# ysbbin/Robust-Object-Detection

Measured on NVIDIA B200. Metric: corrupted images/sec (1360x765 RGB), motion blur k=9, higher is better.
Workload: dtype u8

## Files before the change

robust-object-detection_b200/csrc/api.cu:

```cuda
#include <algorithm>
#include <vector>

#include "rod_internal.h"
#include "rod_tables.h"

using namespace rod;

namespace {

constexpr float kPhiloxMaxSigma = 2048.0f;

bool blur_supported(int k, double angle) { return angle == 0.0 && k >= 1 && k <= 31 && (k & 1) == 1; }

int run_op(rod_plan* plan, int op, const uint8_t* src, uint8_t* dst, const float* noise, float sigma, int k,
           double factor, uint64_t seed, uint64_t first_image, uint32_t offset, const uint8_t* opcodes,
           cudaStream_t stream, int img_lo, int img_hi) {
    switch (op) {
        case ROD_OP_NONE:
            return launch_noise(plan, NOISE_COPY, src, dst, nullptr, nullptr, 0.f, 0, 0, 0, opcodes, ROD_OP_NONE,
                                stream, img_lo, img_hi);
        case ROD_OP_NOISE:
            if (noise == nullptr && sigma > kPhiloxMaxSigma) return ROD_ERR_UNSUPPORTED;
            return launch_noise(plan, noise ? NOISE_COMPAT : NOISE_PHILOX, src, dst, noise, nullptr, sigma, seed,
                                first_image, offset, opcodes, ROD_OP_NOISE, stream, img_lo, img_hi);
        case ROD_OP_BLUR:
            if (plan->f2d_ntaps > 0) return launch_filter2d(plan, src, dst, opcodes, stream, img_lo, img_hi);
            if (!blur_supported(k, 0.0)) return ROD_ERR_UNSUPPORTED;
            if (k == 1)
                return launch_noise(plan, NOISE_COPY, src, dst, nullptr, nullptr, 0.f, 0, 0, 0, opcodes, ROD_OP_BLUR,
                                    stream, img_lo, img_hi);
            return launch_blur(plan, src, dst, k, opcodes, stream, img_lo, img_hi);
        case ROD_OP_LOWRES: {
            int rc = ensure_lowres_tables(plan, factor);
            if (rc != ROD_OK) return rc;
            if (plan->lowres_all_identity)
                return launch_noise(plan, NOISE_COPY, src, dst, nullptr, nullptr, 0.f, 0, 0, 0, opcodes,
                                    ROD_OP_LOWRES, stream, img_lo, img_hi);
            return launch_lowres(plan, src, dst, opcodes, stream, img_lo, img_hi);
        }
        default:
            return ROD_ERR_INVALID_ARG;
    }
}

int run_mixed_ops(rod_plan* plan, int op_lo, const uint8_t* src, uint8_t* dst, const uint8_t* opcodes, const float* noise,
                  float sigma, int k, double factor, uint64_t seed, uint64_t first_image, uint32_t offset,
                  cudaStream_t stream) {
    if (noise == nullptr && sigma > kPhiloxMaxSigma) return ROD_ERR_UNSUPPORTED;
    if (plan->f2d_ntaps == 0 && !blur_supported(k, 0.0)) return ROD_ERR_UNSUPPORTED;
    {
        const int rc = ensure_lowres_tables(plan, factor);
        if (rc != ROD_OK) return rc;
    }
    const bool fork = plan->n_images <= 128;
    if (fork && plan->ev_fork == nullptr) {
        cudaStream_t s2[2] = {nullptr, nullptr};
        cudaEvent_t ef = nullptr, ej[2] = {nullptr, nullptr};
        cudaError_t e = cudaSuccess;
        for (auto& s : s2)
            if (e == cudaSuccess) e = cudaStreamCreateWithFlags(&s, cudaStreamNonBlocking);
        if (e == cudaSuccess) e = cudaEventCreateWithFlags(&ef, cudaEventDisableTiming);
        for (auto& ev : ej)
            if (e == cudaSuccess) e = cudaEventCreateWithFlags(&ev, cudaEventDisableTiming);
        if (e != cudaSuccess) {
            for (auto& s : s2) if (s) cudaStreamDestroy(s);
            if (ef) cudaEventDestroy(ef);
            for (auto& ev : ej) if (ev) cudaEventDestroy(ev);
            return cuda_fail(e);
        }
        plan->aux_streams[0] = s2[0]; plan->aux_streams[1] = s2[1];
        plan->ev_join[0] = ej[0]; plan->ev_join[1] = ej[1];
        plan->ev_fork = ef;
    }
    if (fork) {
        ROD_CUDA(cudaEventRecord(plan->ev_fork, stream));
        for (auto& s : plan->aux_streams) ROD_CUDA(cudaStreamWaitEvent(s, plan->ev_fork, 0));
    }
    int first_rc = ROD_OK;
    for (int op = op_lo; op <= ROD_OP_LOWRES && first_rc == ROD_OK; ++op) {
        cudaStream_t st = stream;
        if (fork && op == ROD_OP_BLUR) st = plan->aux_streams[0];
        if (fork && op == ROD_OP_NOISE) st = plan->aux_streams[1];
        first_rc = run_op(plan, op, src, dst, noise, sigma, k, factor, seed, first_image, offset, opcodes, st, 0, plan->n_images);
    }
    if (fork) {
        for (int i = 0; i < 2; ++i) {
            cudaError_t e = cudaEventRecord(plan->ev_join[i], plan->aux_streams[i]);
            if (e == cudaSuccess) e = cudaStreamWaitEvent(stream, plan->ev_join[i], 0);
            if (e != cudaSuccess && first_rc == ROD_OK) first_rc = cuda_fail(e);
        }
    }
    return first_rc;
}

}

extern "C" const char* rod_version(void) { return "rod_b200 0.1.0 (sm_100a)"; }

extern "C" int rod_device_count(void) {
    int n = 0;
    if (cudaGetDeviceCount(&n) != cudaSuccess) {
        cudaGetLastError();
        return 0;
    }
    return n;
}

extern "C" int rod_last_cuda_error(void) { return g_last_cuda_error; }

extern "C" const char* rod_status_string(int status) {
    switch (status) {
        case ROD_OK: return "ok";
        case ROD_ERR_INVALID_ARG: return "invalid argument";
        case ROD_ERR_UNSUPPORTED: return "parameter outside the exact-parity domain (no approximation, no CPU fallback)";
        case ROD_ERR_CUDA: return "CUDA error";
        case ROD_ERR_NO_DEVICE: return "no CUDA device (there is no CPU fallback)";
        case ROD_ERR_OOM: return "out of memory";
        default: return "unknown status";
    }
}

extern "C" int rod_plan_launches(const rod_plan* plan, int op) {
    if (plan == nullptr) return 0;
    switch (op) {
        case ROD_OP_NONE: case ROD_OP_NOISE: case ROD_OP_BLUR: return 1;
        case ROD_OP_LOWRES: {
            if (plan->d_shapes == nullptr) return 1;
            int n = 0;
            for (int l = 0; l < LR_NUM_LISTS; ++l) n += l != LR_X2_STRIP && plan->lowres[l].n > 0;
            return n > 0 ? n : 1;
        }
        case 100: return 4;
        case 101: return 4;
        default: return 0;
    }
}

extern "C" int rod_noise_u8(const rod_plan* plan, const uint8_t* src, uint8_t* dst, const float* noise, float sigma,
                            uint64_t seed, uint64_t first_image_index, uint32_t offset, const uint8_t* opcodes,
                            void* stream) {
    if (plan == nullptr || src == nullptr || dst == nullptr) return ROD_ERR_INVALID_ARG;
    if (!(sigma >= 0.0f)) return ROD_ERR_INVALID_ARG;
    if (noise == nullptr && sigma > kPhiloxMaxSigma) return ROD_ERR_UNSUPPORTED;
    return launch_noise(plan, noise ? NOISE_COMPAT : NOISE_PHILOX, src, dst, noise, nullptr, sigma, seed,
                        first_image_index, offset, opcodes, ROD_OP_NOISE, (cudaStream_t)stream, 0, plan->n_images);
}

extern "C" int rod_noise_prewarm(int device, float sigma) {
    if (!(sigma >= ROD_GAUSS_TABLE_MIN_SIGMA && sigma <= ROD_GAUSS_TABLE_MAX_SIGMA)) return ROD_OK;
    int prev = 0;
    ROD_CUDA(cudaGetDevice(&prev));
    ROD_CUDA(cudaSetDevice(device));
    const int32_t* t = nullptr;
    const int rc = rod::gauss_table_for(device, sigma, &t);
    cudaSetDevice(prev);
    return rc;
}

extern "C" int rod_gauss_table_i32(float sigma, int32_t* out256) {
    if (out256 == nullptr || !(sigma >= ROD_GAUSS_TABLE_MIN_SIGMA && sigma <= ROD_GAUSS_TABLE_MAX_SIGMA)) return ROD_ERR_INVALID_ARG;
    rod::build_gauss_table(sigma, out256);
    return ROD_OK;
}

extern "C" int rod_plan_set_gaussian_generator(rod_plan* plan, int generator) {
    if (plan == nullptr || (generator != ROD_GAUSS_AUTO && generator != ROD_GAUSS_BOXMULLER && generator != ROD_GAUSS_TABLE_PHILOX7)) return ROD_ERR_INVALID_ARG;
    plan->gauss_generator = generator;
    if (plan->inner != nullptr) plan->inner->gauss_generator = generator;
    return ROD_OK;
}

extern "C" int rod_noise_field_f32(const rod_plan* plan, float* out_field, float sigma, uint64_t seed,
                                   uint64_t first_image_index, uint32_t offset, void* stream) {
    if (plan == nullptr || out_field == nullptr) return ROD_ERR_INVALID_ARG;
    if (!(sigma >= 0.0f) || sigma > kPhiloxMaxSigma) return ROD_ERR_UNSUPPORTED;
    return launch_noise(plan, NOISE_FIELD, nullptr, nullptr, nullptr, out_field, sigma, seed, first_image_index,
                        offset, nullptr, ROD_OP_NOISE, (cudaStream_t)stream, 0, plan->n_images);
}

extern "C" int rod_blur_h_u8(const rod_plan* plan, const uint8_t* src, uint8_t* dst, int k, double angle_deg,
                             const uint8_t* opcodes, void* stream) {
    if (plan == nullptr || src == nullptr || dst == nullptr) return ROD_ERR_INVALID_ARG;
    if (plan->f2d_ntaps > 0 ? (k != plan->f2d_k) : !blur_supported(k, angle_deg)) return ROD_ERR_UNSUPPORTED;
    return run_op(const_cast<rod_plan*>(plan), ROD_OP_BLUR, src, dst, nullptr, 0.f, k, 0.0, 0, 0, 0, opcodes,
                  (cudaStream_t)stream, 0, plan->n_images);
}

extern "C" int rod_lowres_u8(rod_plan* plan, const uint8_t* src, uint8_t* dst, double factor, const uint8_t* opcodes,
                             void* stream) {
    if (plan == nullptr || src == nullptr || dst == nullptr) return ROD_ERR_INVALID_ARG;
    return run_op(plan, ROD_OP_LOWRES, src, dst, nullptr, 0.f, 0, factor, 0, 0, 0, opcodes, (cudaStream_t)stream, 0,
                  plan->n_images);
}

extern "C" int rod_corrupt_batch_u8(rod_plan* plan, const uint8_t* src, uint8_t* dst, const uint8_t* opcodes,
                                    const float* noise, float sigma, int k, double factor, uint64_t seed,
                                    uint64_t first_image_index, uint32_t offset, void* stream) {
    if (plan == nullptr || src == nullptr || dst == nullptr || opcodes == nullptr) return ROD_ERR_INVALID_ARG;
    if (noise == nullptr && sigma > kPhiloxMaxSigma) return ROD_ERR_UNSUPPORTED;
    if (plan->f2d_ntaps == 0 && !blur_supported(k, 0.0)) return ROD_ERR_UNSUPPORTED;
    int rc = ensure_lowres_tables(plan, factor);
    if (rc != ROD_OK) return rc;
    rc = run_op(plan, ROD_OP_NONE, src, dst, noise, sigma, k, factor, seed, first_image_index, offset, opcodes,
                (cudaStream_t)stream, 0, plan->n_images);
    if (rc != ROD_OK) return rc;
    return run_mixed_ops(plan, ROD_OP_NOISE, src, dst, opcodes, noise, sigma, k, factor, seed, first_image_index, offset,
                         (cudaStream_t)stream);
}

extern "C" int rod_corrupt_letterbox_f16(rod_plan* plan, const uint8_t* src, const uint8_t* opcodes, void* out_f16,
                                         int out_h, int out_w, int pad_value, const float* noise, float sigma, int k,
                                         double factor, uint64_t seed, uint64_t first_image_index, uint32_t offset,
                                         void* stream) {
    if (plan == nullptr || src == nullptr || out_f16 == nullptr || opcodes == nullptr) return ROD_ERR_INVALID_ARG;
    if (pad_value < 0 || pad_value > 255) return ROD_ERR_INVALID_ARG;
    struct GeneratorScope {
        rod_plan* p; int saved;
        explicit GeneratorScope(rod_plan* pl) : p(pl), saved(pl->gauss_generator) { p->gauss_generator = ROD_GAUSS_BOXMULLER; }
        ~GeneratorScope() { p->gauss_generator = saved; }
    } generator_scope(plan);
    int rc = ensure_letterbox_tables(plan, out_h, out_w);
    if (rc != ROD_OK) return rc;
    if (plan->d_scratch == nullptr || plan->scratch_bytes < plan->dst_extent) {
        if (plan->d_scratch) cudaFree(plan->d_scratch);
        plan->d_scratch = nullptr;
        ROD_CUDA(cudaMalloc((void**)&plan->d_scratch, plan->dst_extent + 64));
        plan->scratch_bytes = plan->dst_extent;
    }
    const bool fused = plan->lb_all_linear && plan->f2d_ntaps == 0 && blur_supported(k, 0.0) && k >= 3 &&
                       (noise != nullptr || sigma <= kPhiloxMaxSigma);
    if (fused) {
        rc = ensure_lowres_tables(plan, factor);
        if (rc != ROD_OK) return rc;
        const bool in_kernel = plan->lowres_all_x2w && (((uintptr_t)src) & 3) == 0;
        if (!in_kernel) {
            rc = run_op(plan, ROD_OP_LOWRES, src, plan->d_scratch, noise, sigma, k, factor, seed, first_image_index, offset,
                        opcodes, (cudaStream_t)stream, 0, plan->n_images);
            if (rc != ROD_OK) return rc;
        }
        rc = launch_fused_letterbox(plan, src, plan->d_scratch, opcodes, noise, out_f16, pad_value, sigma, k, seed,
                                    first_image_index, offset, in_kernel, (cudaStream_t)stream);
        if (rc != ROD_ERR_UNSUPPORTED) return rc;
    }
    rc = run_mixed_ops(plan, ROD_OP_NOISE, src, plan->d_scratch, opcodes, noise, sigma, k, factor, seed, first_image_index,
                       offset, (cudaStream_t)stream);
    if (rc != ROD_OK) return rc;
    return launch_letterbox(plan, plan->d_scratch, src, opcodes, out_f16, pad_value, (cudaStream_t)stream);
}

extern "C" int rod_resize_linear_u8(const uint8_t* src, int h, int w, int64_t src_pitch, uint8_t* dst, int nh, int nw,
                                    int64_t dst_pitch, void* stream) {
    if (src == nullptr || dst == nullptr || h < 1 || w < 1 || nh < 1 || nw < 1 || src_pitch < 3LL * w || dst_pitch < 3LL * nw ||
        h > 65535 || w > 65535 || nh > 65535 || nw > 65535)
        return ROD_ERR_INVALID_ARG;
    if (nh < h || nw < w) return ROD_ERR_UNSUPPORTED;
    return launch_resize_linear(src, h, w, src_pitch, dst, nh, nw, dst_pitch, (cudaStream_t)stream);
}

extern "C" int rod_restoration_pairs_f32(rod_plan* plan, const uint8_t* src, const uint8_t* flips, const uint8_t* opcodes,
                                         float* corrupted_out, float* clean_out, const float* noise, float sigma, int k,
                                         double factor, uint64_t seed, uint64_t first_image_index, uint32_t offset,
                                         void* stream) {
    if (plan == nullptr || src == nullptr || opcodes == nullptr || corrupted_out == nullptr || clean_out == nullptr)
        return ROD_ERR_INVALID_ARG;
    const int n = plan->n_images;
    for (int i = 1; i < n; ++i)
        if (plan->descs[i].height != plan->descs[0].height || plan->descs[i].width != plan->descs[0].width)
            return ROD_ERR_INVALID_ARG;
    if (plan->inner == nullptr) {
        std::vector<rod_image_desc> d(n);
        const uint64_t bytes = 3ull * plan->descs[0].height * plan->descs[0].width;
        const uint64_t stride = (bytes + 255) / 256 * 256;
        for (int i = 0; i < n; ++i) {
            d[i].src_offset = d[i].dst_offset = i * stride;
            d[i].height = plan->descs[0].height;
            d[i].width = plan->descs[0].width;
            d[i].src_pitch = d[i].dst_pitch = 3ll * d[i].width;
        }
// ... 114 lines not shown
```

robust-object-detection_b200/csrc/blur.cu:

```cuda

#include "rod_internal.h"

namespace rod {

struct BlurParams {
    const DevImage* images;
    const Tile* tiles;
    int n_tiles;
    const uint8_t* src;
    uint8_t* dst;
    const uint8_t* opcodes;
    int k;
    int row_buf_bytes;
    unsigned int* counter;
};

constexpr int kBlurLeft = 64;

__device__ __forceinline__ void cp_async16(uint32_t smem_addr, const void* gptr) {
    asm volatile("cp.async.cg.shared.global [%0], [%1], 16;" ::"r"(smem_addr), "l"(gptr) : "memory");
}
__device__ __forceinline__ void cp_async_wait_all() {
    asm volatile("cp.async.commit_group;\ncp.async.wait_group 0;" ::: "memory");
}
__device__ __forceinline__ void stg16_blur(void* p, uint4 v) {
    asm volatile("st.global.L1::no_allocate.v4.u32 [%0], {%1,%2,%3,%4};" ::"l"(p), "r"(v.x), "r"(v.y), "r"(v.z),
                 "r"(v.w)
                 : "memory");
}

template <int K>
__global__ void __launch_bounds__(256, 4) blur_rows_kernel(BlurParams p) {
    extern __shared__ __align__(16) uint8_t smem[];
    const int warp = threadIdx.x >> 5, lane = threadIdx.x & 31;
    uint8_t* buf = smem + (size_t)warp * p.row_buf_bytes;
    const uint32_t buf_s = (uint32_t)__cvta_generic_to_shared(buf);
    const int k = (K == 0) ? p.k : K;
    const int halo = 3 * (k >> 1);

    for (int sub = 8, ti = 0;;) {
        if (sub >= 8) {
            if (lane == 0) ti = (int)atomicAdd(p.counter, 1u);
            ti = __shfl_sync(0xFFFFFFFFu, ti, 0);
            sub = 0;
        }
        if (ti >= p.n_tiles) break;
        const Tile t = p.tiles[ti];
        const int wr = sub++;
        if (p.opcodes != nullptr && p.opcodes[t.img] != ROD_OP_BLUR) { sub = 8; continue; }
        if (wr >= t.b) { sub = 8; continue; }
        const DevImage im = p.images[t.img];
        const int y = t.a + wr;
        const int n = 3 * im.w;
        const uint8_t* srow = p.src + im.src_off + (int64_t)y * im.src_pitch;
        uint8_t* drow = p.dst + im.dst_off + (int64_t)y * im.dst_pitch;
        const int shift = (int)((uintptr_t)drow & 15);
        uint8_t* row = buf + kBlurLeft + shift;
        const int jf0 = (shift != 0) ? 1 : 0;
        const int jf1 = (n + shift) >> 4;
        const bool right_edge = ((n + shift) & 15) != 0;

        if ((((uintptr_t)srow ^ (uintptr_t)drow) & 15) == 0) {
            const uint8_t* sal = srow - shift;
            for (int j = jf0 + lane; j < jf1; j += 32) cp_async16(buf_s + kBlurLeft + 16 * j, sal + 16 * j);
            const int i = (lane < 16) ? (lane - shift) : (16 * jf1 - shift + lane - 16);
            if (((lane < 16) ? (shift != 0) : right_edge) && i >= 0 && i < n) row[i] = srow[i];
            cp_async_wait_all();
        } else {
            for (int i = lane; i < n; i += 32) row[i] = srow[i];
        }
        __syncwarp();
        if (lane < 2 * halo || K == 0) {
            for (int q = lane; q < 2 * halo; q += 32) {
                const int i = (q < halo) ? (q - halo) : (n + q - halo);
                const int px = (i >= 0) ? i / 3 : -((-i + 2) / 3);
                const int c = i - 3 * px;
                int rp;
                if (im.w > (k >> 1)) rp = (px < 0) ? -px : 2 * (im.w - 1) - px;
                else rp = reflect101(px, im.w);
                row[i] = row[3 * rp + c];
            }
        }
        __syncwarp();
        uint8_t* dal = drow - shift;
        if (K == 9) {
            for (int j = jf0 + lane; j < jf1; j += 32) {
                const uint4* wp = reinterpret_cast<const uint4*>(buf + kBlurLeft + 16 * j - 16);
                const uint4 a = wp[0], b = wp[1], c = wp[2];
                const uint32_t w[12] = {a.x, a.y, a.z, a.w, b.x, b.y, b.z, b.w, c.x, c.y, c.z, c.w};
                uint32_t out[4];
                blur9_chunk16(w, out);
                stg16_blur(dal + 16 * j, make_uint4(out[0], out[1], out[2], out[3]));
            }
            if (lane < 2 && ((lane == 0) ? (shift != 0) : right_edge)) {
                const int j = (lane == 0) ? 0 : jf1;
                const uint4* wp = reinterpret_cast<const uint4*>(buf + kBlurLeft + 16 * j - 16);
                const uint4 a = wp[0], b = wp[1], c = wp[2];
                const uint32_t w[12] = {a.x, a.y, a.z, a.w, b.x, b.y, b.z, b.w, c.x, c.y, c.z, c.w};
                uint32_t out[4];
                blur9_chunk16(w, out);
                const int lo = 16 * j - shift;
                for (int bb = 0; bb < 16; ++bb) {
                    const int i = lo + bb;
                    if (i >= 0 && i < n) drow[i] = (uint8_t)(out[bb >> 2] >> (8 * (bb & 3)));
                }
            }
        } else {
            const int nchunks = (shift + n + 15) >> 4;
            for (int j = lane; j < nchunks; j += 32) {
                const int lo = 16 * j - shift;
                uint32_t out[4];
#pragma unroll
                for (int g = 0; g < 4; ++g) {
                    uint32_t o = 0;
#pragma unroll
                    for (int b = 0; b < 4; ++b) {
                        const int i = lo + 4 * g + b;
                        const uint32_t v = (i >= 0 && i < n) ? blur_byte_generic(row, i, k) : 0u;
                        o |= v << (8 * b);
                    }
                    out[g] = o;
                }
                if (lo >= 0 && lo + 16 <= n) {
                    stg16_blur(dal + 16 * j, make_uint4(out[0], out[1], out[2], out[3]));
                } else {
                    for (int b = 0; b < 16; ++b) {
                        const int i = lo + b;
                        if (i >= 0 && i < n) drow[i] = (uint8_t)(out[b >> 2] >> (8 * (b & 3)));
                    }
                }
            }
        }
        __syncwarp();
    }
}

int launch_blur(const rod_plan* plan, const uint8_t* src, uint8_t* dst, int k, const uint8_t* opcodes,
                cudaStream_t stream, int img_lo, int img_hi) {
    const auto [tiles, n_tiles] = plan->blur_tiles.range(img_lo, img_hi);
    if (n_tiles == 0) return ROD_OK;
    BlurParams p;
    p.images = plan->d_images;
    p.tiles = tiles;
    p.n_tiles = n_tiles;
    p.src = src; p.dst = dst; p.opcodes = opcodes; p.k = k;
    const int row_bytes = 3 * plan->max_w;
    p.row_buf_bytes = kBlurLeft + ((15 + row_bytes + 15) & ~15) + 64;
    int warps = kBlurRowsPerTile;
    while (warps > 1 && (size_t)p.row_buf_bytes * warps > 227 * 1024) --warps;
    const size_t smem = (size_t)p.row_buf_bytes * warps;
    if (smem > 227 * 1024) return ROD_ERR_UNSUPPORTED;
    int ctas_per_sm = (int)((227 * 1024) / (smem + 1024));
    if (ctas_per_sm < 1) ctas_per_sm = 1;
    if (ctas_per_sm > 4) ctas_per_sm = 4;
    p.counter = plan->d_counters + (plan->launch_seq.fetch_add(1u) & (kCounterRing - 1u));
    ROD_CUDA(cudaMemsetAsync(p.counter, 0, sizeof(unsigned int), stream));
    const int grid = grid_for(plan, (p.n_tiles + warps - 1) / warps, ctas_per_sm);
    if (k == 9) {
        ROD_CUDA(cudaFuncSetAttribute(blur_rows_kernel<9>, cudaFuncAttributeMaxDynamicSharedMemorySize, (int)smem));
        blur_rows_kernel<9><<<grid, 32 * warps, smem, stream>>>(p);
    } else {
        ROD_CUDA(cudaFuncSetAttribute(blur_rows_kernel<0>, cudaFuncAttributeMaxDynamicSharedMemorySize, (int)smem));
        blur_rows_kernel<0><<<grid, 32 * warps, smem, stream>>>(p);
    }
    ROD_CUDA(cudaGetLastError());
    return ROD_OK;
}

}
```

robust-object-detection_b200/csrc/plan.cu:

```cuda
#include <map>
#include <new>

#include "rod_internal.h"
#include "rod_tables.h"

namespace rod {

thread_local int g_last_cuda_error = 0;

int grid_for(const rod_plan* plan, int n_tiles, int ctas_per_sm) {
    long long cap = (long long)plan->sm_count * ctas_per_sm;
    return (int)(n_tiles < cap ? n_tiles : cap);
}

static cudaError_t plan_alloc(const rod_plan* plan, void** p, size_t n) {
    const cudaError_t e = block_cache_alloc(plan->device, p, n);
    if (e == cudaSuccess) {
        std::lock_guard<std::mutex> lock(plan->cached_mutex);
        plan->cached_blocks.push_back({*p, n});
    }
    return e;
}
static void plan_free(const rod_plan* plan, void* p) {
    if (p == nullptr) return;
// ... 108 lines not shown
        const DevShape& sh = shapes[plan->h_images[i].shape_id];
        if (odd_image(i)) {
            std::vector<Tile>& list = lists[sh.x2i != 0 ? LR_X2I_CARRY + sh.x2i - 1 : LR_X2G];
            for (int y = 0; y < plan->h_images[i].h; y += band_rows_odd)
                for (int st = 0; st < n_strips(plan->h_images[i].w); ++st)
                    list.push_back(Tile{i, y, std::min(plan->h_images[i].h, y + band_rows_odd), st});
            continue;
        }
        if (sh.strip_rows <= 0) continue;
        if (march_image(i)) {
            const int l = packed_image(i) ? LR_X2P16 + packed_class(i) : regular_image(i) ? LR_X2H16 + packed_class(i)
                          : float_image(i) ? LR_X2F16 + packed_class(i) : al8_image(i) ? LR_X2W8 : LR_X2W4;
            for (int y = 0; y < plan->h_images[i].h; y += band_rows)
                for (int st = 0; st < n_strips(plan->h_images[i].w); ++st)
                    lists[l].push_back(Tile{i, y, std::min(plan->h_images[i].h, y + band_rows), st});
        } else {
            for (int y = 0; y < plan->h_images[i].h; y += sh.strip_rows) lists[LR_X2_REST].push_back(Tile{i, y, 0, 0});
        }
    }
    plan->lowres_factor = -1.0;
    plan_free(plan, plan->d_shapes);
    plan_free(plan, plan->d_tab);
    plan->d_shapes = nullptr;
    plan->d_tab = nullptr;
    int rc = upload(plan, shapes, &plan->d_shapes);
    if (rc == ROD_OK) rc = upload(plan, blob, &plan->d_tab);
    for (int l = 0; l < LR_NUM_LISTS && rc == ROD_OK; ++l) rc = upload_tiles(plan, lists[l], &plan->lowres[l]);
    if (rc != ROD_OK) return rc;
    plan->lowres_x2_smem = x2_smem;
    plan->lowres_factor = factor;
    plan->lowres_all_identity = all_identity;
    plan->lowres_all_x2w = true;
    for (const DevShape& sh : shapes)
        if (!sh.lin_identity && !sh.x2w) plan->lowres_all_x2w = false;
    for (int i = 0; i < plan->n_images; ++i)
        if ((plan->h_images[i].src_pitch & 3) != 0 || (plan->h_images[i].src_off & 3) != 0) plan->lowres_all_x2w = false;
    plan->lowres_half_rows = max_rows;
    plan->lowres_half_cols = max_cols;
    plan->lowres_src_rows = max_src_rows;
    return ROD_OK;
}

int ensure_letterbox_tables(rod_plan* plan, int out_h, int out_w) {
    if (plan->d_lb != nullptr && plan->lb_out_h == out_h && plan->lb_out_w == out_w) return ROD_OK;
    if (out_h < 1 || out_w < 1) return ROD_ERR_INVALID_ARG;
    std::vector<uint32_t> blob;
    std::vector<DevLetterbox> lbs(plan->shapes.size());
    for (size_t s = 0; s < plan->shapes.size(); ++s) {
        DevLetterbox g;
        memset(&g, 0, sizeof(g));
        g.h = plan->shapes[s].h; g.w = plan->shapes[s].w;
        letterbox_geometry(g.h, g.w, out_h, out_w, &g.new_h, &g.new_w, &g.top, &g.left);
        if (g.new_h < 1 || g.new_w < 1 || g.h > 65535 || g.w > 65535) return ROD_ERR_UNSUPPORTED;
        g.identity = (g.new_h == g.h && g.new_w == g.w);
        g.area2 = (!g.identity && g.h == 2 * g.new_h && g.w == 2 * g.new_w);
        if (!g.identity && !g.area2) {
            LinearAxis lx = build_linear_axis(g.w, g.new_w, true);
            LinearAxis ly = build_linear_axis(g.h, g.new_h, false);
            std::vector<uint32_t> ys(g.new_h);
            for (int y = 0; y < g.new_h; ++y) ys[y] = (uint32_t)ly.s0[y] | ((uint32_t)ly.s1[y] << 16);
            g.lx_s0 = blob_push(blob, lx.s0);
            g.lx_a = blob_push(blob, lx.coef);
            g.ly_s = blob_push(blob, ys);
            g.ly_b = blob_push(blob, ly.coef);
            std::vector<uint32_t> pack((size_t)2 * out_w);
            for (int X = 0; X < out_w; ++X) {
                const int cx = X - g.left;
                const bool in = cx >= 0 && cx < g.new_w;
                pack[2 * X] = in ? (uint32_t)(3 * lx.s0[cx]) : 0xFFFFFFFFu;
                pack[2 * X + 1] = in ? lx.coef[cx] : 0u;
            }
            g.lx_pack = blob_push(blob, pack);
            const double stride_words = 2.0 * 3.0 * ((double)g.w / (double)g.new_w) / 4.0;
            g.lane_group = 0;
            for (int pp = 2; pp <= 16; ++pp) {
                const double x = pp * stride_words / 32.0;
                if (fabs(x - nearbyint(x)) * 32.0 < 1.0) { g.lane_group = pp; break; }
            }
        }
        lbs[s] = g;
    }
    if (blob.empty()) blob.push_back(0);
    std::vector<Tile> tiles;
    for (int i = 0; i < plan->n_images; ++i)
        for (int y = 0; y < out_h; y += kLbTH)
            for (int x = 0; x < out_w; x += kLbTW) tiles.push_back(Tile{i, y, x, 0});
    if (plan->d_lb) { plan_free(plan, plan->d_lb); plan->d_lb = nullptr; }
    if (plan->d_lb_tab) { plan_free(plan, plan->d_lb_tab); plan->d_lb_tab = nullptr; }
    int rc = upload(plan, lbs, &plan->d_lb);
    if (rc != ROD_OK) return rc;
    rc = upload(plan, blob, &plan->d_lb_tab);
    if (rc != ROD_OK) return rc;
    rc = upload_tiles(plan, tiles, &plan->lb_tiles);
    if (rc != ROD_OK) return rc;
    plan->lb_all_linear = true;
    for (const DevLetterbox& g : lbs)
        if (g.identity || g.area2) plan->lb_all_linear = false;
    plan->lb_out_h = out_h;
    plan->lb_out_w = out_w;
    return ROD_OK;
}

}

using namespace rod;

extern "C" int rod_plan_create(const rod_image_desc* images, int n_images, rod_plan** out_plan) {
    if (out_plan == nullptr) return ROD_ERR_INVALID_ARG;
    *out_plan = nullptr;
    if (images == nullptr || n_images < 1) return ROD_ERR_INVALID_ARG;
    int ndev = 0;
    if (cudaGetDeviceCount(&ndev) != cudaSuccess || ndev == 0) {
        cudaGetLastError();
        return ROD_ERR_NO_DEVICE;
    }
    rod_plan* plan = new (std::nothrow) rod_plan();
    if (plan == nullptr) return ROD_ERR_OOM;
    cudaError_t e = cudaGetDevice(&plan->device);
    if (e == cudaSuccess) e = cudaDeviceGetAttribute(&plan->sm_count, cudaDevAttrMultiProcessorCount, plan->device);
    if (e != cudaSuccess) { delete plan; return cuda_fail(e); }
    plan->n_images = n_images;
    plan->descs.assign(images, images + n_images);
    plan->h_images.resize(n_images);
    std::map<std::pair<int, int>, int> shape_ids;
    uint64_t elem = 0;
    for (int i = 0; i < n_images; ++i) {
        const rod_image_desc& d = images[i];
        if (d.height < 1 || d.width < 1 || d.width > 65535 || d.height > 65535 || d.src_pitch < 3LL * d.width ||
            d.dst_pitch < 3LL * d.width || (uint64_t)d.height * d.width * 3 > 0x7FFFFFFFull) {
            delete plan;
            return ROD_ERR_INVALID_ARG;
        }
        DevImage& im = plan->h_images[i];
        im.src_off = d.src_offset; im.dst_off = d.dst_offset;
        im.src_pitch = d.src_pitch; im.dst_pitch = d.dst_pitch;
        im.h = d.height; im.w = d.width;
        im.elem_base = elem;
        im.contiguous = (d.src_pitch == 3LL * d.width && d.dst_pitch == 3LL * d.width) ? 1 : 0;
        elem += (uint64_t)d.height * d.width * 3;
        auto key = std::make_pair(d.height, d.width);
        auto it = shape_ids.find(key);
        if (it == shape_ids.end()) {
            it = shape_ids.emplace(key, (int)plan->shapes.size()).first;
            plan->shapes.push_back(HostShape{d.height, d.width});
        }
        im.shape_id = it->second;
        plan->max_w = std::max(plan->max_w, d.width);
        plan->all_contiguous = plan->all_contiguous && im.contiguous;
        plan->src_min_offset = (i == 0) ? d.src_offset : std::min<uint64_t>(plan->src_min_offset, d.src_offset);
        plan->src_extent = std::max<uint64_t>(plan->src_extent, d.src_offset + (uint64_t)(d.height - 1) * d.src_pitch + 3ull * d.width);
        plan->dst_extent = std::max<uint64_t>(plan->dst_extent, d.dst_offset + (uint64_t)(d.height - 1) * d.dst_pitch + 3ull * d.width);
    }
    plan->payload_bytes = elem;
    std::vector<Tile> nt, bt;
    build_noise_tiles(plan->h_images, kNoiseSpan, nt);
    build_blur_tiles(plan->h_images, kBlurRowsPerTile, bt);
    for (int i = 1; i < n_images; ++i) {
        const rod_image_desc& a = images[i - 1];
        const rod_image_desc& b = images[i];
        if (b.src_offset < a.src_offset + (uint64_t)a.height * a.src_pitch - (a.src_pitch - 3ull * a.width) ||
            b.dst_offset < a.dst_offset + (uint64_t)a.height * a.dst_pitch - (a.dst_pitch - 3ull * a.width))
            plan->monotonic = false;
    }
    if (plan_alloc(plan, (void**)&plan->d_counters, kCounterRing * sizeof(unsigned int)) != cudaSuccess) { rod_plan_destroy(plan); return ROD_ERR_OOM; }
    int rc = upload(plan, plan->h_images, &plan->d_images);
    if (rc == ROD_OK) rc = upload_tiles(plan, nt, &plan->noise_tiles);
    if (rc == ROD_OK) rc = upload_tiles(plan, bt, &plan->blur_tiles);
    if (rc != ROD_OK) { rod_plan_destroy(plan); return rc; }
    *out_plan = plan;
    return ROD_OK;
}

extern "C" int rod_set_blur_kernel(rod_plan* plan, const float* kernel, int k) {
    if (plan == nullptr) return ROD_ERR_INVALID_ARG;
    if (kernel == nullptr) {
        plan->f2d_ntaps = 0;
        plan->f2d_k = 0;
        return ROD_OK;
    }
    if (k < 1 || (k & 1) == 0) return ROD_ERR_INVALID_ARG;
    if (k * k >= kF2dMaxElems) return ROD_ERR_UNSUPPORTED;
    std::vector<float4> taps;
    for (int dy = 0; dy < k; ++dy)
        for (int dx = 0; dx < k; ++dx) {
            const float w = kernel[dy * k + dx];
            if (w == 0.0f) continue;
            float4 t;
            const int dxb = 3 * dx;
            memcpy(&t.x, &dy, 4);
            memcpy(&t.y, &dxb, 4);
            t.z = w;
            t.w = 0.f;
            taps.push_back(t);
        }
    if (taps.empty()) return ROD_ERR_INVALID_ARG;
    if (plan->d_f2d_taps) { plan_free(plan, plan->d_f2d_taps); plan->d_f2d_taps = nullptr; }
    int rc = upload(plan, taps, &plan->d_f2d_taps);
    if (rc != ROD_OK) return rc;
    if (plan->f2d_tiles.d == nullptr) {
        std::vector<Tile> tiles;
        build_grid_tiles(plan->h_images, kF2dTH, kF2dTWB, tiles);
        rc = upload_tiles(plan, tiles, &plan->f2d_tiles);
        if (rc != ROD_OK) return rc;
    }
    plan->f2d_ntaps = (int)taps.size();
    plan->f2d_k = k;
    return ROD_OK;
}

extern "C" void rod_plan_destroy(rod_plan* plan) {
    if (plan == nullptr) return;
    if (plan->inner) rod_plan_destroy(plan->inner);
    cudaDeviceSynchronize();
    if (plan->d_patch_clean) cudaFree(plan->d_patch_clean);
    if (plan->d_patch_corrupted) cudaFree(plan->d_patch_corrupted);
    void* ptrs[] = {plan->d_images, plan->noise_tiles.d, plan->blur_tiles.d, plan->d_shapes, plan->d_tab, plan->d_lb,
                    plan->d_lb_tab, plan->lb_tiles.d, plan->d_scratch, plan->d_stage_src, plan->d_f2d_taps,
                    plan->f2d_tiles.d, plan->d_counters, plan->d_stage_dst, plan->d_stage_noise, plan->d_stage_ops};
    for (void* p : ptrs) plan_free(plan, p);
    for (const TileList& l : plan->lowres) plan_free(plan, l.d);
    for (cudaStream_t s : plan->streams)
        if (s) cudaStreamDestroy(s);
    for (cudaStream_t s : plan->aux_streams)
        if (s) cudaStreamDestroy(s);
    for (cudaStream_t s : plan->lr_streams)
        if (s) cudaStreamDestroy(s);
    if (plan->lr_ev_fork) cudaEventDestroy(plan->lr_ev_fork);
    for (cudaEvent_t e : plan->lr_ev_join)
        if (e) cudaEventDestroy(e);
    if (plan->ev_fork) cudaEventDestroy(plan->ev_fork);
    for (cudaEvent_t e : plan->ev_join)
        if (e) cudaEventDestroy(e);
    delete plan;
}

extern "C" int rod_plan_num_images(const rod_plan* plan) { return plan ? plan->n_images : 0; }
extern "C" uint64_t rod_plan_payload_bytes(const rod_plan* plan) { return plan ? plan->payload_bytes : 0; }
```

robust-object-detection_b200/csrc/rod_internal.h:

```cpp
#pragma once
#include <cuda_runtime.h>

#include <atomic>
#include <mutex>
#include <utility>
#include <vector>

#include "../../include/rod_b200.h"
#include "rod_core.h"

namespace rod {

constexpr unsigned int kCounterRing = 4096;

constexpr int kNoiseSpan = 16384;
constexpr int kBlurRowsPerTile = 8;
constexpr int kLowresTH = 32;
constexpr int kLowresTWB = 480;
constexpr int kLbTH = 32;
constexpr int kLbTW = 64;
constexpr int kMaxAreaTaps = 8;
constexpr int kF2dTH = 16;
constexpr int kF2dTWB = 768;
constexpr int kF2dMaxElems = 130;

struct HostShape {
    int h, w;
};

struct DevLetterbox {
    int32_t h, w, new_h, new_w, top, left;
    int32_t area2;
    int32_t identity;
    uint32_t lx_s0, lx_a;
    uint32_t ly_s, ly_b;
    uint32_t lx_pack;
    int32_t lane_group;
};

struct TileList {
    Tile* d = nullptr;
    int n = 0;
    std::vector<int> start;
    std::pair<const Tile*, int> range(int lo, int hi) const {
        if (n == 0) return {d, 0};
        return {d + start[lo], start[hi] - start[lo]};
    }
};

enum LowresList {
    LR_GENERIC,
    LR_X2_STRIP,
    LR_X2_REST,
    LR_X2W8, LR_X2W4,
    LR_X2P16, LR_X2P8, LR_X2P4,
    LR_X2F16, LR_X2F8, LR_X2F4,
    LR_X2H16, LR_X2H8, LR_X2H4,
    LR_X2G,
    LR_X2I_CARRY, LR_X2I_EVEN,
    LR_NUM_LISTS
};

}

struct rod_plan {
    int device = 0;
    int n_images = 0;
    int sm_count = 148;
    std::vector<rod_image_desc> descs;
    std::vector<rod::DevImage> h_images;
    std::vector<rod::HostShape> shapes;
    uint64_t payload_bytes = 0;
    int max_w = 0;
    bool all_contiguous = true;
    uint64_t src_extent = 0, dst_extent = 0;
    uint64_t src_min_offset = 0;

    rod::DevImage* d_images = nullptr;
    rod::TileList noise_tiles, blur_tiles;
    rod::TileList lowres[rod::LR_NUM_LISTS];
    size_t lowres_x2_smem = 0;
    unsigned int* d_counters = nullptr;
    mutable std::atomic<unsigned int> launch_seq{0};
    bool monotonic = true;
    int gauss_generator = ROD_GAUSS_AUTO;

    double lowres_factor = -1.0;
    rod::DevShape* d_shapes = nullptr;
    uint32_t* d_tab = nullptr;
    bool lowres_all_identity = false;
    bool lowres_all_x2w = false;
    int lowres_half_rows = 0, lowres_half_cols = 0;
    int lowres_src_rows = 0;

    int lb_out_h = 0, lb_out_w = 0;
    rod::DevLetterbox* d_lb = nullptr;
    uint32_t* d_lb_tab = nullptr;
    bool lb_all_linear = false;
    rod::TileList lb_tiles;
    uint8_t* d_scratch = nullptr;
    uint64_t scratch_bytes = 0;

    float4* d_f2d_taps = nullptr;
    int f2d_ntaps = 0, f2d_k = 0;
    rod::TileList f2d_tiles;

    rod_plan* inner = nullptr;
    uint8_t* d_patch_clean = nullptr;
    uint8_t* d_patch_corrupted = nullptr;

    uint8_t* d_stage_src = nullptr;
    uint8_t* d_stage_dst = nullptr;
    float* d_stage_noise = nullptr;
    uint8_t* d_stage_ops = nullptr;
    cudaStream_t streams[3] = {nullptr, nullptr, nullptr};
    cudaStream_t aux_streams[2] = {nullptr, nullptr};
    cudaEvent_t ev_fork = nullptr, ev_join[2] = {nullptr, nullptr};
    mutable std::mutex cached_mutex;
    mutable std::vector<std::pair<void*, size_t>> cached_blocks;
    mutable std::mutex lr_mutex;
    mutable cudaStream_t lr_streams[2] = {nullptr, nullptr};
    mutable cudaEvent_t lr_ev_fork = nullptr, lr_ev_join[2] = {nullptr, nullptr};
};

namespace rod {
extern thread_local int g_last_cuda_error;
inline int cuda_fail(cudaError_t e) {
    g_last_cuda_error = (int)e;
    return e == cudaErrorMemoryAllocation ? ROD_ERR_OOM : ROD_ERR_CUDA;
}
#define ROD_CUDA(call)                                  \
    do {                                                \
        cudaError_t _e = (call);                        \
        if (_e != cudaSuccess) return rod::cuda_fail(_e); \
    } while (0)

int grid_for(const rod_plan* plan, int n_tiles, int ctas_per_sm);

cudaError_t block_cache_alloc(int dev, void** p, size_t n);
void block_cache_free(int dev, void* p, size_t n);

int launch_noise(const rod_plan* plan, int mode, const uint8_t* src, uint8_t* dst, const float* noise,
                 float* field_out, float sigma, uint64_t seed, uint64_t first_image, uint32_t offset,
                 const uint8_t* opcodes, int my_op, cudaStream_t stream, int img_lo, int img_hi,
                 int generator = -1 );
int launch_blur(const rod_plan* plan, const uint8_t* src, uint8_t* dst, int k, const uint8_t* opcodes,
                cudaStream_t stream, int img_lo, int img_hi);
int launch_lowres(const rod_plan* plan, const uint8_t* src, uint8_t* dst, const uint8_t* opcodes,
                  cudaStream_t stream, int img_lo, int img_hi);
int launch_filter2d(const rod_plan* plan, const uint8_t* src, uint8_t* dst, const uint8_t* opcodes, cudaStream_t stream,
                    int img_lo, int img_hi);
int launch_gather_patches(const rod_plan* plan, const rod_plan* inner, const uint8_t* src, uint8_t* clean,
                          const uint8_t* flips, cudaStream_t stream);
int launch_resize_linear(const uint8_t* src, int h, int w, int64_t src_pitch, uint8_t* dst, int nh, int nw, int64_t dst_pitch,
                         cudaStream_t stream);
int launch_format_pairs(const rod_plan* inner, const uint8_t* clean, const uint8_t* corrupted, float* clean_out,
                        float* corrupted_out, cudaStream_t stream);
int launch_fused_letterbox(const rod_plan* plan, const uint8_t* src, const uint8_t* scratch, const uint8_t* opcodes,
                           const float* noise, void* out_f16, int pad_value, float sigma, int k, uint64_t seed,
                           uint64_t first_image, uint32_t offset, bool lowres_in_kernel, cudaStream_t stream);
int launch_letterbox(const rod_plan* plan, const uint8_t* img, const uint8_t* src, const uint8_t* opcodes, void* out_f16,
                     int pad_value, cudaStream_t stream);

int gauss_table_for(int device, float sigma, const int32_t** out);
int ensure_lowres_tables(rod_plan* plan, double factor);
int ensure_letterbox_tables(rod_plan* plan, int out_h, int out_w);

enum NoiseMode { NOISE_COMPAT = 0, NOISE_PHILOX = 1, NOISE_COPY = 2, NOISE_FIELD = 3 };
}
```

Before: 946,900.

## Add TMA bulk-copy pipelined blur9 kernel for aligned rows

Adds a k=9 blur kernel that loads whole rows into shared memory with cp.async.bulk and mbarriers. Each warp keeps three row slots in flight so loads overlap compute. Rows are claimed through per-lane atomic counters, with large claims first and pairs of rows at the tail for load balance. The plan now splits blur tiles into bulk-eligible (16-byte aligned, row width within limit) and fallback lists. This adds a second launch when unaligned images exist, plus extra counter-reset logic.

```diff
diff --git a/robust-object-detection_b200/csrc/api.cu b/robust-object-detection_b200/csrc/api.cu
--- a/robust-object-detection_b200/csrc/api.cu
+++ b/robust-object-detection_b200/csrc/api.cu
@@ -123,7 +123,12 @@
 extern "C" int rod_plan_launches(const rod_plan* plan, int op) {
     if (plan == nullptr) return 0;
     switch (op) {
-        case ROD_OP_NONE: case ROD_OP_NOISE: case ROD_OP_BLUR: return 1;
+        case ROD_OP_NONE: case ROD_OP_NOISE: return 1;
+        case ROD_OP_BLUR: {
+            if (plan->f2d_ntaps > 0) return 1;
+            const int n = (plan->blur[BLUR_BULK].n > 0) + (plan->blur[BLUR_ROWS].n > 0);
+            return n > 0 ? n : 1;
+        }
         case ROD_OP_LOWRES: {
             if (plan->d_shapes == nullptr) return 1;
             int n = 0;
diff --git a/robust-object-detection_b200/csrc/blur.cu b/robust-object-detection_b200/csrc/blur.cu
--- a/robust-object-detection_b200/csrc/blur.cu
+++ b/robust-object-detection_b200/csrc/blur.cu
@@ -135,9 +135,148 @@
     }
 }
 
-int launch_blur(const rod_plan* plan, const uint8_t* src, uint8_t* dst, int k, const uint8_t* opcodes,
-                cudaStream_t stream, int img_lo, int img_hi) {
-    const auto [tiles, n_tiles] = plan->blur_tiles.range(img_lo, img_hi);
+constexpr int kBulkWarps = 4;
+constexpr int kBulkSlots = 3;
+constexpr int kBulkPad = 16;
+constexpr int kBulkPairTail = 16;
+constexpr int kBulkHeader = kBulkWarps * kBulkSlots * (8 + 16);
+static_assert(kBulkHeader + kBulkWarps * kBulkSlots * (kBlurBulkMaxRow + 2 * kBulkPad) <= 227 * 1024,
+              "a CTA of the widest BLUR_BULK rows must fit in shared memory");
+
+struct BlurBulkParams {
+    const DevImage* images;
+    const Tile* tiles;
+    int n_rows;
+    int big_claims;
+    const uint8_t* src;
+    uint8_t* dst;
+    const uint8_t* opcodes;
+    int slot_bytes;
+    unsigned int* counter;
+};
+
+struct BulkRow {
+    uint64_t dst_off;
+    int32_t n;
+    int32_t pad;
+};
+
+constexpr uint64_t kHaloLeft = 0x543876BA9EDCull;
+constexpr uint64_t kHaloRight = 0xDEFABC789456ull;
+
+__device__ __forceinline__ void mbar_init(uint32_t bar) {
+    asm volatile("mbarrier.init.shared::cta.b64 [%0], 1;" ::"r"(bar) : "memory");
+}
+__device__ __forceinline__ void mbar_wait(uint32_t bar, uint32_t parity) {
+    asm volatile(
+        "{\n.reg .pred p;\nWAIT:\n"
+        "mbarrier.try_wait.parity.shared::cta.b64 p, [%0], %1;\n"
+        "@!p bra WAIT;\n}" ::"r"(bar), "r"(parity)
+        : "memory");
+}
+__device__ __forceinline__ void bulk_row_load(uint32_t dst, const void* src, uint32_t bytes, uint32_t bar) {
+    asm volatile("mbarrier.arrive.expect_tx.shared::cta.b64 _, [%0], %1;" ::"r"(bar), "r"(bytes) : "memory");
+    asm volatile("cp.async.bulk.shared::cta.global.mbarrier::complete_tx::bytes [%0], [%1], %2, [%3];" ::"r"(dst),
+                 "l"(src), "r"(bytes), "r"(bar)
+                 : "memory");
+}
+
+__global__ void __launch_bounds__(32 * kBulkWarps, 8) blur9_bulk_kernel(BlurBulkParams p) {
+    extern __shared__ __align__(16) uint8_t smem[];
+    const int warp = threadIdx.x >> 5, lane = threadIdx.x & 31;
+    const uint32_t bar0 = (uint32_t)__cvta_generic_to_shared(smem) + 8 * kBulkSlots * warp;
+    BulkRow* rows = reinterpret_cast<BulkRow*>(smem + 8 * kBulkWarps * kBulkSlots) + kBulkSlots * warp;
+    uint8_t* slot0 = smem + kBulkHeader + (size_t)p.slot_bytes * kBulkSlots * warp;
+    const uint32_t slot0_s = (uint32_t)__cvta_generic_to_shared(slot0);
+
+    unsigned int next = 0;
+    unsigned int* const claims = p.counter + lane;
+    int row = 0, end = 0;
+    bool exhausted = false;
+    Tile t;
+    DevImage im;
+    auto next_row = [&](const uint8_t** src_row, uint64_t* dst_off) -> int {
+        for (;;) {
+            if (row == end) {
+                if (exhausted) return 0;
+                const int c = (int)next;
+                row = (c < p.big_claims) ? kBlurRowsPerTile * c : kBlurRowsPerTile * p.big_claims + 2 * (c - p.big_claims);
+                if (row >= p.n_rows) { exhausted = true; end = row; return 0; }
+                end = row + ((c < p.big_claims) ? kBlurRowsPerTile : 2);
+                next = atomicAdd(claims, 1u);
+                t = p.tiles[row / kBlurRowsPerTile];
+                if (p.opcodes != nullptr && p.opcodes[t.img] != ROD_OP_BLUR) { row = end; continue; }
+                im = p.images[t.img];
+            }
+            const int r = row++ % kBlurRowsPerTile;
+            if (r >= t.b) { row = end; continue; }
+            const int y = t.a + r;
+            *src_row = p.src + im.src_off + (int64_t)y * im.src_pitch;
+            *dst_off = im.dst_off + (uint64_t)((int64_t)y * im.dst_pitch);
+            return 3 * im.w;
+        }
+    };
+    auto issue = [&](int s, int n, const uint8_t* src_row, uint64_t dst_off) {
+        rows[s].dst_off = dst_off;
+        rows[s].n = n;
+        if (n > 0) bulk_row_load(slot0_s + s * p.slot_bytes + kBulkPad, src_row, (uint32_t)n, bar0 + 8 * s);
+    };
+    if (lane == 0) {
+        for (int s = 0; s < kBulkSlots; ++s) mbar_init(bar0 + 8 * s);
+        asm volatile("fence.mbarrier_init.release.cluster;" ::: "memory");
+        next = atomicAdd(claims, 1u);
+        for (int s = 0; s < kBulkSlots; ++s) {
+            const uint8_t* src_row = nullptr;
+            uint64_t dst_off = 0;
+            const int n = next_row(&src_row, &dst_off);
+            issue(s, n, src_row, dst_off);
+        }
+    }
+    for (int s = 0, phase = 0;;) {
+        __syncwarp();
+        const BulkRow r = rows[s];
+        if (r.n == 0) break;
+        uint8_t* srow = slot0 + s * p.slot_bytes + kBulkPad;
+        mbar_wait(bar0 + 8 * s, phase);
+        if (lane < 24) {
+            const int q = (lane < 12) ? lane : lane - 12;
+            const int from = (lane < 12) ? (int)((kHaloLeft >> (4 * q)) & 15) : r.n - (int)((kHaloRight >> (4 * q)) & 15);
+            srow[(lane < 12) ? q - 12 : r.n + q] = srow[from];
+        }
+        __syncwarp();
+        uint8_t* drow = p.dst + r.dst_off;
+        for (int j = lane; j < (r.n >> 4); j += 32) {
+            const uint4* wp = reinterpret_cast<const uint4*>(srow + 16 * j - 16);
+            const uint4 a = wp[0], b = wp[1], c = wp[2];
+            const uint32_t w[12] = {a.x, a.y, a.z, a.w, b.x, b.y, b.z, b.w, c.x, c.y, c.z, c.w};
+            uint32_t out[4];
+            blur9_chunk16(w, out);
+            stg16_blur(drow + 16 * j, make_uint4(out[0], out[1], out[2], out[3]));
+        }
+        __syncwarp();
+        const uint8_t* src_row = nullptr;
+        uint64_t dst_off = 0;
+        int n = 0;
+        if (lane == 0) n = next_row(&src_row, &dst_off);
+        if (__shfl_sync(0xFFFFFFFFu, n > r.n, 0)) asm volatile("fence.proxy.async.shared::cta;" ::: "memory");
+        __syncwarp();
+        if (lane == 0) issue(s, n, src_row, dst_off);
+        if (++s == kBulkSlots) { s = 0; phase ^= 1; }
+    }
+    __syncthreads();
+    if (threadIdx.x == 0) {
+        __threadfence();
+        if (atomicAdd(p.counter + 1, 1u) == gridDim.x - 1) {
+            p.counter[0] = 0u;
+            p.counter[1] = 0u;
+        }
+    }
+}
+
+namespace {
+int launch_blur_rows(const rod_plan* plan, const TileList& list, const uint8_t* src, uint8_t* dst, int k,
+                     const uint8_t* opcodes, cudaStream_t stream, int img_lo, int img_hi) {
+    const auto [tiles, n_tiles] = list.range(img_lo, img_hi);
     if (n_tiles == 0) return ROD_OK;
     BlurParams p;
     p.images = plan->d_images;
@@ -167,4 +306,36 @@
     return ROD_OK;
 }
 
-}
+int launch_blur_bulk(const rod_plan* plan, const uint8_t* src, uint8_t* dst, const uint8_t* opcodes,
+                     cudaStream_t stream, int img_lo, int img_hi) {
+    const auto [tiles, n_tiles] = plan->blur[BLUR_BULK].range(img_lo, img_hi);
+    if (n_tiles == 0) return ROD_OK;
+    BlurBulkParams p;
+    p.images = plan->d_images;
+    p.tiles = tiles;
+    p.n_rows = kBlurRowsPerTile * n_tiles;
+    p.big_claims = n_tiles - n_tiles / kBulkPairTail;
+    p.src = src; p.dst = dst; p.opcodes = opcodes;
+    p.slot_bytes = plan->blur_bulk_row + 2 * kBulkPad;
+    const size_t smem = kBulkHeader + (size_t)p.slot_bytes * kBulkSlots * kBulkWarps;
+    int ctas_per_sm = (int)((227 * 1024) / (smem + 1024));
+    ctas_per_sm = ctas_per_sm < 1 ? 1 : (ctas_per_sm > 8 ? 8 : ctas_per_sm);
+    p.counter = plan->d_counters + kCounterRing + 2 * (plan->launch_seq.fetch_add(1u) & (kCounterRing - 1u));
+    ROD_CUDA(cudaFuncSetAttribute(blur9_bulk_kernel, cudaFuncAttributeMaxDynamicSharedMemorySize, (int)smem));
+    blur9_bulk_kernel<<<grid_for(plan, (n_tiles + kBulkWarps - 1) / kBulkWarps, ctas_per_sm), 32 * kBulkWarps, smem,
+                        stream>>>(p);
+    ROD_CUDA(cudaGetLastError());
+    return ROD_OK;
+}
+}
+
+int launch_blur(const rod_plan* plan, const uint8_t* src, uint8_t* dst, int k, const uint8_t* opcodes,
+                cudaStream_t stream, int img_lo, int img_hi) {
+    if (k != 9 || (((uintptr_t)src | (uintptr_t)dst) & 15) != 0)
+        return launch_blur_rows(plan, plan->blur[BLUR_ALL], src, dst, k, opcodes, stream, img_lo, img_hi);
+    const int rc = launch_blur_bulk(plan, src, dst, opcodes, stream, img_lo, img_hi);
+    if (rc != ROD_OK) return rc;
+    return launch_blur_rows(plan, plan->blur[BLUR_ROWS], src, dst, k, opcodes, stream, img_lo, img_hi);
+}
+
+}
diff --git a/robust-object-detection_b200/csrc/plan.cu b/robust-object-detection_b200/csrc/plan.cu
--- a/robust-object-detection_b200/csrc/plan.cu
+++ b/robust-object-detection_b200/csrc/plan.cu
@@ -284,9 +284,17 @@
         plan->dst_extent = std::max<uint64_t>(plan->dst_extent, d.dst_offset + (uint64_t)(d.height - 1) * d.dst_pitch + 3ull * d.width);
     }
     plan->payload_bytes = elem;
-    std::vector<Tile> nt, bt;
+    std::vector<Tile> nt, bt, blur_lists[BLUR_NUM_LISTS];
     build_noise_tiles(plan->h_images, kNoiseSpan, nt);
     build_blur_tiles(plan->h_images, kBlurRowsPerTile, bt);
+    for (const Tile& t : bt) {
+        const DevImage& im = plan->h_images[t.img];
+        const uint64_t a = im.src_off | im.dst_off | (uint64_t)im.src_pitch | (uint64_t)im.dst_pitch | (uint64_t)(3 * im.w);
+        const bool bulk = (a & 15) == 0 && 3 * im.w <= kBlurBulkMaxRow;
+        blur_lists[bulk ? BLUR_BULK : BLUR_ROWS].push_back(t);
+        blur_lists[BLUR_ALL].push_back(t);
+        if (bulk) plan->blur_bulk_row = std::max(plan->blur_bulk_row, 3 * im.w);
+    }
     for (int i = 1; i < n_images; ++i) {
         const rod_image_desc& a = images[i - 1];
         const rod_image_desc& b = images[i];
@@ -294,10 +302,13 @@
             b.dst_offset < a.dst_offset + (uint64_t)a.height * a.dst_pitch - (a.dst_pitch - 3ull * a.width))
             plan->monotonic = false;
     }
-    if (plan_alloc(plan, (void**)&plan->d_counters, kCounterRing * sizeof(unsigned int)) != cudaSuccess) { rod_plan_destroy(plan); return ROD_ERR_OOM; }
-    int rc = upload(plan, plan->h_images, &plan->d_images);
+    const size_t counter_bytes = 3 * kCounterRing * sizeof(unsigned int);
+    if (plan_alloc(plan, (void**)&plan->d_counters, counter_bytes) != cudaSuccess) { rod_plan_destroy(plan); return ROD_ERR_OOM; }
+    const cudaError_t ze = cudaMemset(plan->d_counters, 0, counter_bytes);
+    int rc = ze == cudaSuccess ? ROD_OK : cuda_fail(ze);
+    if (rc == ROD_OK) rc = upload(plan, plan->h_images, &plan->d_images);
     if (rc == ROD_OK) rc = upload_tiles(plan, nt, &plan->noise_tiles);
-    if (rc == ROD_OK) rc = upload_tiles(plan, bt, &plan->blur_tiles);
+    for (int l = 0; l < BLUR_NUM_LISTS && rc == ROD_OK; ++l) rc = upload_tiles(plan, blur_lists[l], &plan->blur[l]);
     if (rc != ROD_OK) { rod_plan_destroy(plan); return rc; }
     *out_plan = plan;
     return ROD_OK;
@@ -346,10 +357,11 @@
     cudaDeviceSynchronize();
     if (plan->d_patch_clean) cudaFree(plan->d_patch_clean);
     if (plan->d_patch_corrupted) cudaFree(plan->d_patch_corrupted);
-    void* ptrs[] = {plan->d_images, plan->noise_tiles.d, plan->blur_tiles.d, plan->d_shapes, plan->d_tab, plan->d_lb,
+    void* ptrs[] = {plan->d_images, plan->noise_tiles.d, plan->d_shapes, plan->d_tab, plan->d_lb,
                     plan->d_lb_tab, plan->lb_tiles.d, plan->d_scratch, plan->d_stage_src, plan->d_f2d_taps,
                     plan->f2d_tiles.d, plan->d_counters, plan->d_stage_dst, plan->d_stage_noise, plan->d_stage_ops};
     for (void* p : ptrs) plan_free(plan, p);
+    for (const TileList& l : plan->blur) plan_free(plan, l.d);
     for (const TileList& l : plan->lowres) plan_free(plan, l.d);
     for (cudaStream_t s : plan->streams)
         if (s) cudaStreamDestroy(s);
diff --git a/robust-object-detection_b200/csrc/rod_internal.h b/robust-object-detection_b200/csrc/rod_internal.h
--- a/robust-object-detection_b200/csrc/rod_internal.h
+++ b/robust-object-detection_b200/csrc/rod_internal.h
@@ -15,6 +15,7 @@
 
 constexpr int kNoiseSpan = 16384;
 constexpr int kBlurRowsPerTile = 8;
+constexpr int kBlurBulkMaxRow = 19200;
 constexpr int kLowresTH = 32;
 constexpr int kLowresTWB = 480;
 constexpr int kLbTH = 32;
@@ -61,6 +62,13 @@
     LR_NUM_LISTS
 };
 
+enum BlurList {
+    BLUR_BULK,
+    BLUR_ROWS,
+    BLUR_ALL,
+    BLUR_NUM_LISTS
+};
+
 }
 
 struct rod_plan {
@@ -77,7 +85,9 @@
     uint64_t src_min_offset = 0;
 
     rod::DevImage* d_images = nullptr;
-    rod::TileList noise_tiles, blur_tiles;
+    rod::TileList noise_tiles;
+    rod::TileList blur[rod::BLUR_NUM_LISTS];
+    int blur_bulk_row = 0;
     rod::TileList lowres[rod::LR_NUM_LISTS];
     size_t lowres_x2_smem = 0;
     unsigned int* d_counters = nullptr;
```

Measured after the change: 986,000 (median of 6 runs). 1.04x the previous value.
